# yangt1013/SPEINet

Measured on AMD Instinct MI355X. Metric: deblurred 720p frames/sec, higher is better.
Workload: dtype f16 (correlation top2)

## Files before the change

### include/speinet_hip.h

```cpp
#ifndef SPEINET_HIP_H
#define SPEINET_HIP_H

#include <stdint.h>

#ifdef __cplusplus
extern "C" {
#endif

typedef void* spei_stream_t;

#define SPEI_ACT_NONE 0
#define SPEI_ACT_RELU 1
#define SPEI_ACT_GELU 2

#define SPEI_F32 0
#define SPEI_BF16 1
#define SPEI_F16 2

#define SPEI_CONV 0
#define SPEI_CONV_TRANSPOSED 1

int spei_version(void);
const char* spei_last_error(void);
const char* spei_arch(void);
// ... 10 lines not shown
                   int W, int Cin, spei_stream_t stream);

int spei_igemm_f32(const float* a0, int lda0, int k0, const float* a1, int lda1, int k1, const float* w,
                   const float* bias, float* out, int ldo, const float* residual, int ldr,
                   const float* rowscale, int Hin, int Win, int Hout, int Wout, int N, int ksize, int stride,
                   int pad, int mode, int act, spei_stream_t stream);

int spei_igemm_f32_batched(const float* a0, int lda0, int k0, const float* a1, int lda1, int k1, const float* w,
                           const float* bias, float* out, int ldo, const float* residual, int ldr,
                           const float* rowscale, int Hin, int Win, int Hout, int Wout, int N, int ksize, int stride,
                           int pad, int mode, int act, int batch, spei_stream_t stream);

int spei_conv_slab16(int fmt, const void* a0, int lda0, int k0, const void* a1, int lda1, int k1, int a_fmt,
                     const void* wfrag_hi, const void* wfrag_lo, const float* bias, void* out, int ldo, int out_fmt,
                     const float* residual, int ldr, const float* rowscale, int Hin, int Win, int Hout, int Wout,
                     int N, int ksize, int stride, int pad, int act, int ln_input, spei_stream_t stream);

int spei_conv_slab16_batched(int fmt, const void* a0, int k0, int a_fmt, const void* wfrag, const void* wfrag_lo, const float* bias,
                             void* out, int out_fmt, const float* residual, int batch, int Hin, int Win, int Hout, int Wout, int N,
                             int ksize, int stride, int pad, int act, spei_stream_t stream);

int spei_conv32_ws16(int fmt, const void* a, int a_fmt, const void* wfrag, const float* bias, void* out, int out_fmt, int batch,
                     int H, int W, int act, spei_stream_t stream);

int spei_conv64_ws16(int fmt, const void* a, int a_fmt, const void* wfrag, const float* bias, void* out, int out_fmt, int batch,
                     int H, int W, int act, spei_stream_t stream);

int spei_mlp_fused16(int fmt, const float* x, float* out, const void* w1_frag, const float* b1, const void* w2_frag,
                     const float* b2, int64_t M, spei_stream_t stream);

int spei_convt2_slab16(int fmt, const void* a0, int lda0, int k0, int a_fmt, const void* wfrag00, const void* wfrag01,
                       const void* wfrag10, const void* wfrag11, const float* bias, void* out, int ldo, int out_fmt,
                       int Hin, int Win, int N, int act, spei_stream_t stream);

int spei_convt2_slab16x3(const float* a0, int lda0, int k0, const void* const* whi4, const void* const* wlo4, const float* bias,
                         float* out, int ldo, int Hin, int Win, int N, int act, spei_stream_t stream);

int spei_conv3x3_256_pipe16(int fmt, const float* x, const void* w_frag, const float* bias, const float* residual, float* out,
                            int batch, int H, int W, spei_stream_t stream);

int spei_conv5_out_slab16(int fmt, const void* in, int ldi, int in_fmt, const void* wfrag, const float* bias32, float* out_chw,
                          int H, int W, spei_stream_t stream);

int spei_attn_fused16(int fmt, const float* x, float* out, const void* yhat, const void* wq_frag, const float* bq,
                      const void* wkv_frag, const float* bkv, const void* wproj_frag, const float* bproj,
                      const float* relbias, int H, int W, int shift, spei_stream_t stream);
// ... 233 lines not shown
```

### speinet_amd/csrc/common.h

```cpp
#pragma once
#include <hip/hip_runtime.h>
#include <stdint.h>
#include <stdio.h>
#include "../../include/speinet_hip.h"

void spei_set_error(const char* fmt, ...);

#define SPEI_REQUIRE(cond, ...)            \
    do {                                   \
        if (!(cond)) {                     \
            spei_set_error(__VA_ARGS__);   \
            return -1;                     \
        }                                  \
    } while (0)

#define SPEI_CHECK_LAUNCH(name)                                                          \
    do {                                                                                 \
        hipError_t e__ = hipGetLastError();                                              \
        if (e__ != hipSuccess) {                                                         \
            spei_set_error("%s: launch failed: %s", name, hipGetErrorString(e__));       \
            return -2;                                                                   \
        }                                                                                \
    } while (0)

// ... 108 lines not shown
__device__ __forceinline__ typename lpv<LP>::x4 to_lp4(f32x4 v) {
    typename lpv<LP>::x4 h;
    h[0] = to_lp<LP>(v[0]); h[1] = to_lp<LP>(v[1]); h[2] = to_lp<LP>(v[2]); h[3] = to_lp<LP>(v[3]);
    return h;
}
typedef unsigned u32x4 __attribute__((ext_vector_type(4)));

template <int CTRL>
__device__ __forceinline__ float dpp_quad(float v) {
    return __int_as_float(__builtin_amdgcn_update_dpp(0, __float_as_int(v), CTRL, 0xF, 0xF, true));
}
__device__ __forceinline__ void quad_transpose4(float& a0, float& a1, float& a2, float& a3, int t) {
    const bool b0 = t & 1, b1 = t & 2;
    float s = b0 ? a0 : a1, r = dpp_quad<0xB1>(s);
    if (b0) a0 = r; else a1 = r;
    s = b0 ? a2 : a3; r = dpp_quad<0xB1>(s);
    if (b0) a2 = r; else a3 = r;
    s = b1 ? a0 : a2; r = dpp_quad<0x4E>(s);
    if (b1) a0 = r; else a2 = r;
    s = b1 ? a1 : a3; r = dpp_quad<0x4E>(s);
    if (b1) a1 = r; else a3 = r;
}

__device__ __forceinline__ float spei_gray_px(float r, float g, float b) {
    return __fmaf_rn(0.114f, b, __fmaf_rn(0.2989f, r, 0.587f * g)) / 255.0f;
}
```

### speinet_amd/csrc/conv32_ws16.hip

```cpp
#include "common.h"

namespace {

constexpr int C = 32, KS = 5, PAD = 2, NTAP = KS * KS;
constexpr int TH = 16, TW = 32;
constexpr int IH = TH + KS - 1, IW = TW + KS - 1;
constexpr int PITCH = 2 * C + 16;
constexpr int SLAB = IH * IW * PITCH;
constexpr int NTHR = 256, RT = 4;

struct WsParams {
    const void* a;
    const void* wfrag;
    const float* bias;
    void* out;
    int H, W, batch, act;
    int tiles_x, tiles_y, total;
    long long* stamps;
};

__device__ __forceinline__ void mfma_aw(f32x16& acc, const lpv<_Float16>::x8& w, const lpv<_Float16>::x8& b) {
    asm volatile("v_mfma_f32_32x32x16_f16 %0, %1, %2, %0" : "+v"(acc) : "a"(w), "v"(b));
}
__device__ __forceinline__ void mfma_aw(f32x16& acc, const lpv<__bf16>::x8& w, const lpv<__bf16>::x8& b) {
    asm volatile("v_mfma_f32_32x32x16_bf16 %0, %1, %2, %0" : "+v"(acc) : "a"(w), "v"(b));
}

template <typename TA> struct Chunk { static constexpr int CPP = sizeof(TA) == 4 ? 8 : 4; };

template <typename LP, typename TA, typename TO>
__global__ __launch_bounds__(NTHR, 1) void conv32_ws_kernel(const WsParams p) {
    typedef typename lpv<LP>::x8 lp8;
    typedef typename lpv<LP>::x4 lp4;
    constexpr int CPP = Chunk<TA>::CPP;
    constexpr int NCH = IH * IW * CPP;
    constexpr int NIT = (NCH + NTHR - 1) / NTHR;
    constexpr int NPH = sizeof(TA) == 4 ? 2 : 1;
    constexpr int NITH = (NIT + NPH - 1) / NPH;
    extern __shared__ __attribute__((aligned(16))) unsigned char smem[];

    const int tid = threadIdx.x, lane = tid & 63, wave = tid >> 6;
    const int fr = lane & 31, fk = lane >> 5;

    lp8 wreg[NTAP][2];
    {
        const LP* wp = static_cast<const LP*>(p.wfrag) + lane * 8;
#pragma unroll
        for (int t = 0; t < NTAP; ++t)
#pragma unroll
            for (int s = 0; s < 2; ++s) wreg[t][s] = *reinterpret_cast<const lp8*>(wp + (t * 2 + s) * 512);
    }
    float biasv[16];
#pragma unroll
    for (int r = 0; r < 16; ++r) biasv[r] = p.bias ? p.bias[8 * (r >> 2) + 4 * fk + (r & 3)] : 0.f;

    typedef u32x4 stage_t;
    stage_t sreg[NITH];
    const size_t map_elems = (size_t)p.H * p.W * C;
    const int per_map = p.tiles_x * p.tiles_y;

    auto tile_origin = [&](int t, int& b, int& oy0, int& ox0) {
        b = t / per_map;
        const int r = t - b * per_map;
        const int ty = r / p.tiles_x;
        oy0 = ty * TH;
        ox0 = (r - ty * p.tiles_x) * TW;
    };
    constexpr int PPI = NTHR / CPP, E = 16 / (int)sizeof(TA);
    const int p0 = tid / CPP, sub = tid - p0 * CPP;
    const int iy0 = p0 / IW, ix0 = p0 - iy0 * IW;
    const int lds0 = p0 * PITCH + sub * (sizeof(TA) == 4 ? 8 : 16);
    auto advance = [](int& iy, int& ix) {
        ix += PPI % IW;
        iy += PPI / IW;
        if (ix >= IW) { ix -= IW; ++iy; }
    };
    auto load_slab = [&](int t, int ph) {
        int b, oy0, ox0;
        tile_origin(t, b, oy0, ox0);
        const TA* base = static_cast<const TA*>(p.a) + (size_t)b * map_elems + sub * E;
// ... 11 lines not shown
    auto store_slab = [&](int t, int buf, int ph, int lo, int hi) {
        int b, oy0, ox0;
        tile_origin(t, b, oy0, ox0);
        unsigned char* sl = smem + buf * SLAB + lds0;
        int iy = iy0, ix = ix0;
#pragma unroll
        for (int it = 0; it < NIT; ++it) {
            if (it >= ph * NITH + lo && it < ph * NITH + hi && it < (ph + 1) * NITH && iy < IH) {
                const int j = it - ph * NITH;
                const bool ok = ((unsigned)(oy0 - PAD + iy) < (unsigned)p.H) & ((unsigned)(ox0 - PAD + ix) < (unsigned)p.W);
                if constexpr (sizeof(TA) == 4) {
                    const f32x4 v = __builtin_bit_cast(f32x4, sreg[j]);
                    lp4 h = to_lp4<LP>(v);
                    if (!ok) h = lp4{(LP)0.f, (LP)0.f, (LP)0.f, (LP)0.f};
                    *reinterpret_cast<lp4*>(sl + it * PPI * PITCH) = h;
                } else {
                    *reinterpret_cast<stage_t*>(sl + it * PPI * PITCH) = ok ? sreg[j] : stage_t{0u, 0u, 0u, 0u};
                }
            }
            advance(iy, ix);
        }
    };

    int t = blockIdx.x;
    if (t >= p.total) return;
#pragma unroll
    for (int ph = 0; ph < NPH; ++ph) {
        load_slab(t, ph);
        store_slab(t, 0, ph, 0, NITH);
    }
    lds_barrier();

    int boff[RT];
#pragma unroll
    for (int i = 0; i < RT; ++i) boff[i] = ((wave * RT + i) * IW + fr) * PITCH + fk * 16;

    int buf = 0;
    for (; t < p.total; t += gridDim.x, buf ^= 1) {
        const int tn = t + gridDim.x;
        const bool more = tn < p.total;
        const int tl = more ? tn : t;
        const bool st_ = t == (int)blockIdx.x + (int)gridDim.x;
        if (st_) SPEI_STAMP(p.stamps, 0);
        load_slab(tl, 0);
        if (st_) SPEI_STAMP(p.stamps, 1);
        __builtin_amdgcn_sched_barrier(0);

        const unsigned char* sl = smem + buf * SLAB;
        f32x16 acc[RT];
#pragma unroll
        for (int i = 0; i < RT; ++i)
#pragma unroll
            for (int r = 0; r < 16; ++r) acc[i][r] = biasv[r];
        lp8 bq[3][RT];
        auto step_off = [](int step) { const int tap = step >> 1; return ((tap / KS) * IW + (tap % KS)) * PITCH + (step & 1) * 32; };
#pragma unroll
        for (int d = 0; d < 2; ++d)
#pragma unroll
            for (int i = 0; i < RT; ++i) bq[d][i] = *reinterpret_cast<const lp8*>(sl + boff[i] + step_off(d));
#pragma unroll
        for (int step = 0; step < NTAP * 2; ++step) {
            const int tap = step >> 1, s2 = step & 1;
            if (step + 2 < NTAP * 2) {
#pragma unroll
                for (int i = 0; i < RT; ++i) bq[(step + 2) % 3][i] = *reinterpret_cast<const lp8*>(sl + boff[i] + step_off(step + 2));
            }
#pragma unroll
            for (int i = 0; i < RT; ++i) mfma_aw(acc[i], wreg[tap][s2], bq[step % 3][i]);
            if (NPH == 2 && step == NTAP) {
                store_slab(tl, buf ^ 1, 0, 0, NITH);
                load_slab(tl, 1);
            }
            if (NPH == 1 && step >= NTAP && ((step - NTAP) & 1) == 0 && (step - NTAP) / 2 < NITH)
                store_slab(tl, buf ^ 1, 0, (step - NTAP) / 2, (step - NTAP) / 2 + 1);
        }

        if (st_) SPEI_STAMP(p.stamps, 2);
        {
            int b, oy0, ox0;
            tile_origin(t, b, oy0, ox0);
            TO* ob = static_cast<TO*>(p.out) + (size_t)b * map_elems;
            const int ox = ox0 + fr;
#pragma unroll
            for (int i = 0; i < RT; ++i) {
                const int oy = oy0 + wave * RT + i;
                if (oy < p.H && ox < p.W) {
                    TO* o = ob + ((size_t)oy * p.W + ox) * C + 4 * fk;
#pragma unroll
                    for (int g = 0; g < 4; ++g) {
                        f32x4 v = {acc[i][4 * g], acc[i][4 * g + 1], acc[i][4 * g + 2], acc[i][4 * g + 3]};
                        if (p.act == SPEI_ACT_RELU) v = f32x4{fmaxf(v[0], 0.f), fmaxf(v[1], 0.f), fmaxf(v[2], 0.f), fmaxf(v[3], 0.f)};
                        if constexpr (sizeof(TO) == 4) *reinterpret_cast<f32x4*>(o + 8 * g) = v;
                        else *reinterpret_cast<lp4*>(o + 8 * g) = to_lp4<LP>(v);
                    }
                }
            }
        }
        if (st_) SPEI_STAMP(p.stamps, 3);
        if (NPH == 2) store_slab(tl, buf ^ 1, 1, 0, NITH);
        else store_slab(tl, buf ^ 1, 0, (NTAP + 1) / 2, NITH);
        if (st_) SPEI_STAMP(p.stamps, 4);
        lds_barrier();
        if (st_) SPEI_STAMP(p.stamps, 5);
    }
}

template <typename LP>
int launch_ws(const WsParams& p, int a16, int o16, hipStream_t st) {
    const size_t lds = 2 * (size_t)SLAB;
    const int cus = spei_num_cus();
    const dim3 grid(p.total < cus ? p.total : cus);
    if (a16 && o16) {
        ensure_dyn_lds<&conv32_ws_kernel<LP, LP, LP>>(lds);
        hipLaunchKernelGGL((conv32_ws_kernel<LP, LP, LP>), grid, dim3(NTHR), lds, st, p);
    } else if (!a16 && o16) {
        ensure_dyn_lds<&conv32_ws_kernel<LP, float, LP>>(lds);
        hipLaunchKernelGGL((conv32_ws_kernel<LP, float, LP>), grid, dim3(NTHR), lds, st, p);
    } else if (a16 && !o16) {
        ensure_dyn_lds<&conv32_ws_kernel<LP, LP, float>>(lds);
        hipLaunchKernelGGL((conv32_ws_kernel<LP, LP, float>), grid, dim3(NTHR), lds, st, p);
    } else {
        ensure_dyn_lds<&conv32_ws_kernel<LP, float, float>>(lds);
        hipLaunchKernelGGL((conv32_ws_kernel<LP, float, float>), grid, dim3(NTHR), lds, st, p);
    }
    return 0;
}

}

extern "C" int spei_conv32_ws16(int fmt, const void* a, int a_fmt, const void* wfrag, const float* bias, void* out, int out_fmt, int batch,
                                int H, int W, int act, spei_stream_t stream) {
    SPEI_REQUIRE(a && wfrag && out, "spei_conv32_ws16: null pointer");
    SPEI_REQUIRE((fmt == SPEI_BF16 || fmt == SPEI_F16) && (a_fmt == SPEI_F32 || a_fmt == fmt) && (out_fmt == SPEI_F32 || out_fmt == fmt),
                 "spei_conv32_ws16: fmt=%d a_fmt=%d out_fmt=%d", fmt, a_fmt, out_fmt);
    SPEI_REQUIRE(batch >= 1 && H > 0 && W > 0 && (int64_t)batch * cdiv(H, TH) * cdiv(W, TW) < (1ll << 30) && (int64_t)H * W < (1ll << 26),
                 "spei_conv32_ws16: batch=%d of %dx%d", batch, H, W);
    SPEI_REQUIRE(act == SPEI_ACT_NONE || act == SPEI_ACT_RELU, "spei_conv32_ws16: act=%d", act);
    SPEI_REQUIRE(((uintptr_t)a | (uintptr_t)wfrag | (uintptr_t)out) % 16 == 0 && a != out, "spei_conv32_ws16: 16-byte alignment, out must not be the input");
    WsParams p;
    p.a = a; p.wfrag = wfrag; p.bias = bias; p.out = out; p.H = H; p.W = W; p.batch = batch; p.act = act;
    p.tiles_x = cdiv(W, TW); p.tiles_y = cdiv(H, TH); p.total = batch * p.tiles_x * p.tiles_y;
    p.stamps = spei_stamp_buffer();
    hipStream_t st = (hipStream_t)stream;
    const int a16 = a_fmt != SPEI_F32, o16 = out_fmt != SPEI_F32;
    const int rc = fmt == SPEI_F16 ? launch_ws<_Float16>(p, a16, o16, st) : launch_ws<__bf16>(p, a16, o16, st);
    if (rc) return rc;
    SPEI_CHECK_LAUNCH("spei_conv32_ws16");
    return 0;
}
```

### speinet_amd/csrc/resblock.hip

```cpp
#include "common.h"

namespace {

constexpr int GATE_TR16 = 16;
constexpr int GATE_TR32 = 8;
__host__ __device__ inline int gate_tr(bool lp) { return lp ? GATE_TR16 : GATE_TR32; }
__host__ __device__ inline int gate_tc(int C) { return 256 / (C / 8); }

struct GateWs {
    float* rowpmax;
    float* rowpsum;
    float* colpmax;
    float* colpsum;
    float* tilesum;
    int ntx, nty;
};
__host__ __device__ inline GateWs carve(float* ws, int H, int W, int C, bool lp) {
    GateWs g;
    g.ntx = (W + gate_tc(C) - 1) / gate_tc(C);
    g.nty = (H + gate_tr(lp) - 1) / gate_tr(lp);
    g.rowpmax = ws;
    g.rowpsum = g.rowpmax + (size_t)g.ntx * H * C;
    g.colpmax = g.rowpsum + (size_t)g.ntx * H * C;
    g.colpsum = g.colpmax + (size_t)g.nty * W * C;
// ... 287 lines not shown
                }
            }
        }
        g2[i] = fmaf(acc, hc_bn[0], hc_bn[1]);
    }
}

template <typename T>
__global__ __launch_bounds__(256) void resblock_apply_kernel(const float* __restrict__ x, const T* __restrict__ x1,
                                                             const float* __restrict__ s, const float* __restrict__ g1,
                                                             const float* __restrict__ g2, const float* __restrict__ extra,
                                                             float* __restrict__ out, int ldo, int H, int W, int C) {
    const int cg = C / 4;
    const int64_t total = (int64_t)H * W * cg;
    {
        const size_t b = blockIdx.y;
        x += b * H * W * C; x1 += b * H * W * C; out += b * H * W * ldo;
        s += b * C; g1 += b * H * C; g2 += b * W * C;
    }
    for (int64_t i = (int64_t)blockIdx.x * 256 + threadIdx.x; i < total; i += (int64_t)gridDim.x * 256) {
        const int c = (int)(i % cg) * 4;
        const int64_t pix = i / cg;
        const int xx = (int)(pix % W), yy = (int)(pix / W);
        const float4 a = *reinterpret_cast<const float4*>(x + pix * C + c);
        const f32x4 bv = ld4<T>(x1 + pix * C + c);
        const float4 b = make_float4(bv[0], bv[1], bv[2], bv[3]);
        const float4 sv = *reinterpret_cast<const float4*>(s + c);
        const float4 u = *reinterpret_cast<const float4*>(g1 + (size_t)yy * C + c);
        const float4 v = *reinterpret_cast<const float4*>(g2 + (size_t)xx * C + c);
        float4 o;
        o.x = (b.x * sv.x + (b.x * u.x + b.x * v.x)) + a.x;
        o.y = (b.y * sv.y + (b.y * u.y + b.y * v.y)) + a.y;
        o.z = (b.z * sv.z + (b.z * u.z + b.z * v.z)) + a.z;
        o.w = (b.w * sv.w + (b.w * u.w + b.w * v.w)) + a.w;
        if (extra) {
            const float4 e = *reinterpret_cast<const float4*>(extra + pix * C + c);
            o.x += e.x; o.y += e.y; o.z += e.z; o.w += e.w;
        }
        *reinterpret_cast<float4*>(out + pix * ldo + c) = o;
    }
}

}

extern "C" int64_t spei_gate_ws_floats(int H, int W, int C) {
    if (C != 32 && C != 64 && C != 128) return 0;
    const int64_t ntx = (W + gate_tc(C) - 1) / gate_tc(C), nty = (H + GATE_TR32 - 1) / GATE_TR32;
    return 2 * ntx * H * C + 2 * nty * W * C + ntx * nty * C;
}

static int resblock_gates_run(const void* x1, int x1_fmt, int batch, int H, int W, int C, const float* se_w1, const float* se_b1,
                              const float* se_w2, const float* se_b2, const float* cw_w, const float* cw_bn,
                              const float* hc_w, const float* hc_bn, float* s, float* g1, float* g2, float* ws,
                              spei_stream_t stream) {
    SPEI_REQUIRE(batch >= 1 && batch <= 65535, "spei_resblock_gates_batched: batch=%d", batch);
    SPEI_REQUIRE(x1 && se_w1 && se_b1 && se_w2 && se_b2 && cw_w && cw_bn && hc_w && hc_bn && s && g1 && g2 && ws,
                 "spei_resblock_gates: null pointer");
    SPEI_REQUIRE(C == 32 || C == 64 || C == 128, "spei_resblock_gates: C=%d (32/64/128 built)", C);
    SPEI_REQUIRE(H > 0 && W > 0, "spei_resblock_gates: empty map");
    SPEI_REQUIRE(((uintptr_t)x1 | (uintptr_t)ws) % 16 == 0, "spei_resblock_gates: 16-byte alignment required");
    hipStream_t st = (hipStream_t)stream;
    SPEI_REQUIRE(x1_fmt == SPEI_F32 || x1_fmt == SPEI_BF16 || x1_fmt == SPEI_F16, "spei_resblock_gates: x1_fmt=%d", x1_fmt);
// ... 64 lines not shown
```

### speinet_amd/engine.py

```python
from __future__ import annotations

import contextlib
from functools import partial

import torch

from .ops import ACT_GELU, ACT_RELU, CONV_T, BMap, Ctx, FMap


def _resblocks(ctx: Ctx, f: FMap, blocks, extra=None, out=None) -> FMap:
    n = len(blocks)
    for i, pk in enumerate(blocks):
        last = i == n - 1
        f = ctx.resblock(f, pk, extra=extra if last else None, out=out if last else None)
    return f


def in_block(ctx: Ctx, frame: torch.Tensor, pk: dict) -> FMap:
    ctx = ctx.for_stage("enc")
    return _resblocks(ctx, ctx.conv5_in(frame, pk["head_w"], pk["head_b"]), pk["blocks"])


def enc_stage(ctx: Ctx, f: FMap, pk: dict, extra=None, out=None) -> FMap:
    ctx = ctx.for_stage("enc")
    n = pk["head_b"].numel()
    f = ctx.igemm(f, pk["head_w"], pk["head_b"], n, ksize=5, stride=2, act=ACT_RELU)
    return _resblocks(ctx, f, pk["blocks"], extra, out)


def enc(ctx: Ctx, frame: torch.Tensor, P: dict, extra=None, out=None) -> FMap:
    return enc_stage(ctx, enc_stage(ctx, in_block(ctx, frame, P["inBlock"]), P["encoder_first"]), P["encoder_second"], extra, out)


def enc_batched(ctx: Ctx, frames: list, P: dict):
    ctx = ctx.for_stage("enc")
    assert ctx.batched_available()
    b, (h, w) = len(frames), frames[0].shape[-2:]
    ib = P["inBlock"]
    lv1 = BMap.empty(b, h, w, ib["head_b"].numel(), frames[0].device)
    lib_in = lambda i: ctx.conv5_in(frames[i], ib["head_w"], ib["head_b"], out=lv1.map(i))
    for i in range(b):
        lib_in(i)
    for pk in ib["blocks"]:
        lv1 = ctx.resblock_batched(lv1, pk)
    levels = [lv1]
    f = lv1
    for name in ("encoder_first", "encoder_second"):
        st = P[name]
        f = ctx.igemm_batched(f, st["head_w"], st["head_b"], st["head_b"].numel(), 5, stride=2, act=ACT_RELU)
        for pk in st["blocks"]:
            f = ctx.resblock_batched(f, pk)
        levels.append(f)
    return levels


def dec_stage(ctx: Ctx, f: FMap, pk: dict) -> FMap:
    f = _resblocks(ctx, f, pk["blocks"])
    return ctx.for_stage("convt").igemm(f, pk["tail_w"], pk["tail_b"], pk["tail_b"].numel(), ksize=3, stride=2, mode=CONV_T, act=ACT_RELU)


class SwinX:

    def __init__(self, ctx: Ctx, f_mid: FMap, sw: dict):
        ctx = ctx.for_stage("swin")
        self.f_mid = f_mid
        self.x_first = ctx.igemm(f_mid, sw["conv_first_w"], sw["conv_first_b"], 256, ksize=3)
        self.xt0 = ctx.layernorm(self.x_first.t, sw["pe_g"], sw["pe_b"])
# ... 358 lines not shown
```

### speinet_amd/ops.py

```python
from __future__ import annotations

import ctypes as C
import dataclasses
from typing import Optional

import numpy as np
import torch

from . import _lib, y4m
from . import light as _light
from .pack import BF16, F16, F32, LP_DTYPE, PackedW, fmt_of

ACT_NONE, ACT_RELU, ACT_GELU = 0, 1, 2
CONV, CONV_T = 0, 1

PRECISIONS = ("f32", "bf16x3", "bf16", "f16")
CORR_PRECISIONS = ("bf16x3", "single", "top2")
_CORR_ALIASES = {"bf16": "single", "bf16r": "top2", "f16": "single"}


class FMap:
    __slots__ = ("t", "H", "W", "C", "ld", "off")

    def __init__(self, t: torch.Tensor, H: int, W: int, C_: int, off: int = 0):
# ... 34 lines not shown
        return FMap(x.permute(1, 2, 0).reshape(h * w, c).contiguous().float(), h, w, c)


class BMap:
    __slots__ = ("t", "B", "H", "W", "C")

    def __init__(self, t: torch.Tensor, B: int, H: int, W: int, C_: int):
        assert t.is_cuda and t.is_contiguous() and t.shape == (B * H * W, C_)
        self.t, self.B, self.H, self.W, self.C = t, B, H, W, C_

    @staticmethod
    def empty(B: int, H: int, W: int, C_: int, device, dtype=torch.float32) -> "BMap":
        return BMap(torch.empty(B * H * W, C_, device=device, dtype=dtype), B, H, W, C_)

    @property
    def fmt(self) -> int:
        return fmt_of(self.t.dtype)

    def map(self, b: int) -> FMap:
        n = self.H * self.W
        return FMap(self.t[b * n:(b + 1) * n], self.H, self.W, self.C)


def _vp(p) -> C.c_void_p:
    return C.c_void_p(p)


class _timed:
    def __init__(self, ctx: "Ctx", name: str):
        self.on = ctx.profile is not None and name in ctx.profile
        self.ctx, self.name = ctx, name

    def __enter__(self):
        if self.on:
            self.s = torch.cuda.Event(enable_timing=True)
            self.e = torch.cuda.Event(enable_timing=True)
            self.s.record(torch.cuda.current_stream(self.ctx.device))
        return self

    def __exit__(self, *a):
        if self.on:
            self.e.record(torch.cuda.current_stream(self.ctx.device))
            self.ctx.profile[self.name].append((self.s, self.e))
        return False


def _tensor_bytes(x) -> int:
    t = x.t if hasattr(x, "t") else x
    return t.numel() * t.element_size() if torch.is_tensor(t) else 0


def _conv_sub(method: str, a, k, out):
    if method == "conv5_in":
        return "level1", 2.0 * 25 * 3 * 32 * a[0].shape[-2] * a[0].shape[-1], _tensor_bytes(a[0]) + _tensor_bytes(out)
    if method == "conv5_out":
        return "level1", 2.0 * 25 * 32 * 3 * a[0].H * a[0].W, _tensor_bytes(a[0]) + 12 * a[0].H * a[0].W
    src, n = a[0], a[3]
    ks = a[4] if len(a) > 4 else k.get("ksize", 1)
    if n == 32 and src.C == 32 and ks == 5 and k.get("stride", a[5] if len(a) > 5 else 1) == 1:
        maps = getattr(src, "B", 1)
        return "level1", 2.0 * 25 * 32 * 32 * maps * src.H * src.W, _tensor_bytes(src) + _tensor_bytes(out)
    return "rest", 0.0, 0


def _family(name: str):
    def deco(fn):
        def wrapper(self, *a, **k):
            pr = self.profile
            if pr is None or "families" not in pr:
                return fn(self, *a, **k)
            st = torch.cuda.current_stream(self.device)
            s_, e_ = torch.cuda.Event(enable_timing=True), torch.cuda.Event(enable_timing=True)
            s_.record(st)
            out = fn(self, *a, **k)
            e_.record(st)
            pr["families"].setdefault(name, []).append((s_, e_))
            if name == "conv":
                sub, fl, by = _conv_sub(fn.__name__, a, k, out)
                rec = pr.setdefault("conv_sub", {}).setdefault(sub, {"events": [], "flops": 0.0, "bytes": 0})
# ... 304 lines not shown

@dataclasses.dataclass(frozen=True, slots=True, eq=False)
class Ctx:
    ACT_NONE, ACT_RELU, ACT_GELU = ACT_NONE, ACT_RELU, ACT_GELU
    CONV, CONV_T = CONV, CONV_T
    SPLIT_STAGES = ("glue", "dec2")

    precision: str = "f32"
    corr_precision: str = "bf16x3"
    device: Optional[torch.device] = None
    bf16_storage: bool = True
    x1_bf16: bool = True
    fuse_mlp: bool = True
    fuse_attn: bool = True
    commute_upconv: bool = True
    commute_any: bool = False
    corr_bf16: bool = True
    corr_diag: bool = True
    split_decode: bool = True
    batch_enc: bool = True
    attn_win4: bool = True
    conv32_ws: bool = True
    conv64_ws: Optional[bool] = None
    conv3_pipe: bool = True
    stage: Optional[dict] = None
    profile: Optional[dict] = None
    capture: Optional[dict] = None

    def __post_init__(self):
        put = object.__setattr__
        if self.precision not in PRECISIONS:
            raise ValueError(f"unknown precision {self.precision!r}")
        put(self, "corr_precision", _CORR_ALIASES.get(self.corr_precision, self.corr_precision))
        if self.corr_precision not in CORR_PRECISIONS:
            raise ValueError(f"unknown correlation precision {self.corr_precision!r}")
        cur = torch.cuda.current_device() if torch.cuda.is_available() else 0
        device = torch.device("cuda", cur) if self.device is None else torch.device(self.device)
        if device.type != "cuda":
            raise RuntimeError("speinet_amd runs on MI355X only (HIP kernels); there is no CPU path")
        put(self, "device", torch.device("cuda", cur) if device.index is None else device)
        for k in _BOOL_KNOBS:
            if type(getattr(self, k)) is not bool:
                put(self, k, bool(getattr(self, k)))
        if self.conv64_ws is not None:
            put(self, "conv64_ws", bool(self.conv64_ws))
        put(self, "stage", dict(self.stage) if self.stage else {})
# ... 196 lines not shown
            w = PackedW(w.reshape(1, *w.shape), x.device)
        n = w.shape[1]
        if out is None:
            out = torch.empty(m, n, device=x.device, dtype=out_dtype)
        self.igemm(FMap(x, m, 1, k), w, b, n, act=act, ln_input=ln_input,
                   residual=FMap(residual, m, 1, n) if residual is not None else None, out=FMap(out, m, 1, n))
        return out

    @_family("streaming")
    def resblock_gates(self, x1: FMap, pk: dict):
        dev = x1.t.device
        lib = _lib.lib()
        tp = self._tp
        assert x1.off == 0 and x1.ld == x1.C
        s = torch.empty(x1.C, device=dev)
        g1 = torch.empty(x1.H, x1.C, device=dev)
        g2 = torch.empty(x1.W, x1.C, device=dev)
        ws = torch.empty(lib.spei_gate_ws_floats(x1.H, x1.W, x1.C), device=dev)
        _lib.check(lib.spei_resblock_gates(self._fp(x1), x1.fmt, x1.H, x1.W, x1.C, tp(pk["se_w1"]), tp(pk["se_b1"]), tp(pk["se_w2"]),
                                           tp(pk["se_b2"]), tp(pk["cw_w"]), tp(pk["cw_bn"]), tp(pk["hc_w"]), tp(pk["hc_bn"]),
                                           tp(s), tp(g1), tp(g2), tp(ws), self._stream()), "spei_resblock_gates")
        return s, g1, g2

    def resblock(self, x: FMap, pk: dict, extra: Optional[FMap] = None, out: Optional[FMap] = None) -> FMap:
        idt = self.inter_dtype()
        c = x.C
        assert x.off == 0 and x.ld == c
        t = self.igemm(x, pk["w1"], pk["b1"], c, ksize=5, act=ACT_RELU, out_dtype=idt)
        x1 = self.igemm(t, pk["w2"], pk["b2"], c, ksize=5, out_dtype=idt if self.x1_bf16 else torch.float32)
        s, g1, g2 = self.resblock_gates(x1, pk)
        if out is None:
            out = FMap.empty(x.H, x.W, c, x.t.device)
        if extra is not None:
            assert extra.off == 0 and extra.ld == c
        self._apply(x, x1, s, g1, g2, extra, out, c)
        return out

    @_family("streaming")
    def _apply(self, x, x1, s, g1, g2, extra, out, c):
        _lib.check(_lib.lib().spei_resblock_apply(self._fp(x), self._fp(x1), x1.fmt, self._tp(s), self._tp(g1), self._tp(g2),
                                                  self._fp(extra), self._fp(out), out.ld, x.H, x.W, c, self._stream()),
                   "spei_resblock_apply")

    def batched_available(self) -> bool:
        return self.batched_kernels() and self.x1_bf16 and self.bf16_storage and self.batch_enc

    def conv32_ws_available(self) -> bool:
        return self.lp16 and self.conv32_ws

    def conv64_ws_available(self) -> bool:
        return self.lp16 and (self.conv32_ws if self.conv64_ws is None else self.conv64_ws)

    def batched_kernels(self) -> bool:
        return self.lp16

    @_family("conv")
    def igemm_batched(self, a: BMap, w, bias: torch.Tensor, N: int, ksize: int, stride: int = 1, act: int = ACT_NONE,
                      out_dtype=torch.float32, residual: Optional[BMap] = None, out: Optional[BMap] = None) -> BMap:
        assert self.batched_kernels() and not torch.is_tensor(w) and w.fhi is not None
        pad = ksize // 2
        ho, wo = (a.H + 2 * pad - ksize) // stride + 1, (a.W + 2 * pad - ksize) // stride + 1
        assert tuple(w.shape) == (ksize * ksize, N, a.C) and a.t.dtype in (torch.float32, LP_DTYPE[self.fmt])
        if out is None:
            out = BMap.empty(a.B, ho, wo, N, a.t.device, out_dtype)
        assert (out.B, out.H, out.W, out.C) == (a.B, ho, wo, N) and out.t.data_ptr() != a.t.data_ptr()
        if residual is not None:
            assert (residual.B, residual.H, residual.W, residual.C) == (a.B, ho, wo, N) and residual.t.dtype == torch.float32
            assert residual.t.data_ptr() != a.t.data_ptr()
        tp = self._tp
        if self._persistent_conv(a, w, bias, N, ksize, stride, act, residual, out, a.B):
            return out
        _lib.check(_lib.lib().spei_conv_slab16_batched(self.fmt, tp(a.t), a.C, a.fmt, tp(w.frag(self.fmt)), _vp(0), tp(bias), tp(out.t), out.fmt,
                                                       tp(residual.t) if residual is not None else _vp(0), a.B, a.H, a.W, ho, wo, N, ksize,
                                                       stride, pad, act, self._stream()),
                   "spei_conv_slab16_batched")
        return out

    def resblock_batched(self, x: BMap, pk: dict) -> BMap:
        idt = self.inter_dtype()
        c, dev = x.C, x.t.device
        lib = _lib.lib()
        tp = self._tp
        t = self.igemm_batched(x, pk["w1"], pk["b1"], c, 5, act=ACT_RELU, out_dtype=idt)
        x1 = self.igemm_batched(t, pk["w2"], pk["b2"], c, 5, out_dtype=idt)
        del t
        return self._gates_apply_batched(x, x1, pk)

    @_family("streaming")
    def _gates_apply_batched(self, x: BMap, x1: BMap, pk: dict) -> BMap:
        c, dev = x.C, x.t.device
        lib = _lib.lib()
        tp = self._tp
        s = torch.empty(x.B, c, device=dev)
        g1 = torch.empty(x.B, x.H, c, device=dev)
        g2 = torch.empty(x.B, x.W, c, device=dev)
        ws = torch.empty(x.B * lib.spei_gate_ws_floats(x.H, x.W, c), device=dev)
        _lib.check(lib.spei_resblock_gates_batched(tp(x1.t), x1.fmt, x.B, x.H, x.W, c, tp(pk["se_w1"]), tp(pk["se_b1"]), tp(pk["se_w2"]),
                                                   tp(pk["se_b2"]), tp(pk["cw_w"]), tp(pk["cw_bn"]), tp(pk["hc_w"]), tp(pk["hc_bn"]),
                                                   tp(s), tp(g1), tp(g2), tp(ws), self._stream()), "spei_resblock_gates_batched")
        out = BMap.empty(x.B, x.H, x.W, c, dev)
        _lib.check(lib.spei_resblock_apply_batched(tp(x.t), tp(x1.t), x1.fmt, tp(s), tp(g1), tp(g2), tp(out.t), x.B, x.H, x.W, c,
                                                   self._stream()), "spei_resblock_apply_batched")
        return out

    def ln_fused_available(self) -> bool:
        return self.precision != "f32"

    def attn_fused_available(self) -> bool:
        return self.lp16 and self.fuse_attn and self.bf16_storage

    def mlp_fused_available(self) -> bool:
        return self.lp16 and self.fuse_mlp

    def swin_multi_available(self) -> bool:
        return self.attn_fused_available() and self.attn_win4 and self.mlp_fused_available() and self.batched_kernels()

    @_family("swin")
    def attn_fused(self, x: torch.Tensor, yhat: torch.Tensor, bk: dict, H: int, W: int, shift: int, out: torch.Tensor) -> torch.Tensor:
        assert x.shape[0] % (H * W) == 0 and x.shape[1] == 256 and x.dtype == torch.float32 and out.shape == x.shape and out.dtype == torch.float32
        f = self.fmt
        assert yhat.shape == x.shape and yhat.dtype == LP_DTYPE[f]
        tp = self._tp
# ... 136 lines not shown
```

Baseline: 41.27.

## Fuse resblock gated-apply into next block's first conv32 weight-stationary kernel

Defers the resblock gate-apply (x + x1*(s+g1+g2)) so that the next resblock's first 5x5 conv computes it on the fly while staging its input slab. The gated sum is written to LDS as the conv input and also stored to global as the new residual x. The staging goes through a register ring, and gate vectors are double-buffered in LDS. This removes one full-resolution streaming kernel and its read-then-reread of x per resblock. In exchange the conv loader reads more bytes per pixel (fp32 x plus x1 and the gate rows), register pressure rises, and the gated sum is recomputed on halo pixels.

Measured after the change: 41.63, median of 6. No clear change (+0.9%).

```diff
diff --git a/include/speinet_hip.h b/include/speinet_hip.h
--- a/include/speinet_hip.h
+++ b/include/speinet_hip.h
@@ -56,6 +56,9 @@
 
 int spei_conv32_ws16(int fmt, const void* a, int a_fmt, const void* wfrag, const float* bias, void* out, int out_fmt, int batch,
                      int H, int W, int act, spei_stream_t stream);
+
+int spei_conv32_ws16_gated(int fmt, const float* x, const void* x1, const float* s, const float* g1, const float* g2, const void* wfrag,
+                           const float* bias, float* xo, void* t, int batch, int H, int W, int act, spei_stream_t stream);
 
 int spei_conv64_ws16(int fmt, const void* a, int a_fmt, const void* wfrag, const float* bias, void* out, int out_fmt, int batch,
                      int H, int W, int act, spei_stream_t stream);
diff --git a/speinet_amd/csrc/common.h b/speinet_amd/csrc/common.h
--- a/speinet_amd/csrc/common.h
+++ b/speinet_amd/csrc/common.h
@@ -154,6 +154,17 @@
     if (b1) a1 = r; else a3 = r;
 }
 
+__device__ __forceinline__ f32x4 spei_gated_sum4(f32x4 x, f32x4 x1, f32x4 s, f32x4 g1, f32x4 g2) {
+#pragma clang fp contract(off)
+    f32x4 o;
+#pragma unroll
+    for (int e = 0; e < 4; ++e) {
+        const float p2 = x1[e] * g2[e];
+        o[e] = __builtin_fmaf(x1[e], s[e], __builtin_fmaf(x1[e], g1[e], p2)) + x[e];
+    }
+    return o;
+}
+
 __device__ __forceinline__ float spei_gray_px(float r, float g, float b) {
     return __fmaf_rn(0.114f, b, __fmaf_rn(0.2989f, r, 0.587f * g)) / 255.0f;
 }
diff --git a/speinet_amd/csrc/conv32_ws16.hip b/speinet_amd/csrc/conv32_ws16.hip
--- a/speinet_amd/csrc/conv32_ws16.hip
+++ b/speinet_amd/csrc/conv32_ws16.hip
@@ -8,6 +8,9 @@
 constexpr int PITCH = 2 * C + 16;
 constexpr int SLAB = IH * IW * PITCH;
 constexpr int NTHR = 256, RT = 4;
+constexpr int G2_OFF = IH * C * 4, GS_OFF = G2_OFF + IW * C * 4, GATE = GS_OFF + C * 4;
+constexpr int NGC = GATE / 16;
+constexpr int BIAS_OFF = 2 * SLAB + 2 * GATE;
 
 struct WsParams {
     const void* a;
@@ -17,7 +20,14 @@
     int H, W, batch, act;
     int tiles_x, tiles_y, total;
     long long* stamps;
+    const void* x1;
+    const float* s;
+    const float* g1;
+    const float* g2;
+    float* xo;
 };
+
+typedef unsigned u32x2 __attribute__((ext_vector_type(2)));
 
 __device__ __forceinline__ void mfma_aw(f32x16& acc, const lpv<_Float16>::x8& w, const lpv<_Float16>::x8& b) {
     asm volatile("v_mfma_f32_32x32x16_f16 %0, %1, %2, %0" : "+v"(acc) : "a"(w), "v"(b));
@@ -28,8 +38,9 @@
 
 template <typename TA> struct Chunk { static constexpr int CPP = sizeof(TA) == 4 ? 8 : 4; };
 
-template <typename LP, typename TA, typename TO>
+template <typename LP, typename TA, typename TO, bool GATED = false>
 __global__ __launch_bounds__(NTHR, 1) void conv32_ws_kernel(const WsParams p) {
+    static_assert(!GATED || sizeof(TA) == 4, "gated input: x is fp32");
     typedef typename lpv<LP>::x8 lp8;
     typedef typename lpv<LP>::x4 lp4;
     constexpr int CPP = Chunk<TA>::CPP;
@@ -37,6 +48,7 @@
     constexpr int NIT = (NCH + NTHR - 1) / NTHR;
     constexpr int NPH = sizeof(TA) == 4 ? 2 : 1;
     constexpr int NITH = (NIT + NPH - 1) / NPH;
+    constexpr int RING = 8;
     extern __shared__ __attribute__((aligned(16))) unsigned char smem[];
 
     const int tid = threadIdx.x, lane = tid & 63, wave = tid >> 6;
@@ -53,9 +65,17 @@
     float biasv[16];
 #pragma unroll
     for (int r = 0; r < 16; ++r) biasv[r] = p.bias ? p.bias[8 * (r >> 2) + 4 * fk + (r & 3)] : 0.f;
+    if constexpr (GATED) {
+#pragma unroll
+        for (int g = 0; g < 4; ++g)
+            if (fr == 0 && wave == 0)
+                *reinterpret_cast<f32x4*>(smem + BIAS_OFF + (8 * g + 4 * fk) * 4) = f32x4{biasv[4 * g], biasv[4 * g + 1], biasv[4 * g + 2], biasv[4 * g + 3]};
+    }
 
     typedef u32x4 stage_t;
-    stage_t sreg[NITH];
+    stage_t sreg[GATED ? RING : NITH];
+    u32x2 s1reg[GATED ? RING : 1];
+    stage_t greg[2];
     const size_t map_elems = (size_t)p.H * p.W * C;
     const int per_map = p.tiles_x * p.tiles_y;
 
@@ -113,12 +133,80 @@
         }
     };
 
+    int p0t = p0;
+    auto load_chunk = [&](int t, int it, int slot) {
+        int b, oy0, ox0;
+        tile_origin(t, b, oy0, ox0);
+        const int pix = p0t + it * PPI, iy = min(pix / IW, IH - 1), ix = pix - (pix / IW) * IW;
+        const int gy = min(max(oy0 - PAD + iy, 0), p.H - 1), gx = min(max(ox0 - PAD + ix, 0), p.W - 1);
+        const size_t off = (size_t)b * map_elems + sub * E + (gy * p.W + gx) * C;
+        sreg[slot] = *reinterpret_cast<const stage_t*>(static_cast<const float*>(p.a) + off);
+        s1reg[slot] = *reinterpret_cast<const u32x2*>(static_cast<const LP*>(p.x1) + off);
+    };
+    auto store_chunk = [&](int t, int buf, int it, int slot, bool wr) {
+        int b, oy0, ox0;
+        tile_origin(t, b, oy0, ox0);
+        const int pix = p0t + it * PPI, iy = pix / IW, ix = pix - iy * IW;
+        if (iy < IH) {
+            const unsigned char* gt = smem + 2 * SLAB + buf * GATE + sub * 16;
+            const bool ok = ((unsigned)(oy0 - PAD + iy) < (unsigned)p.H) & ((unsigned)(ox0 - PAD + ix) < (unsigned)p.W);
+            const lp4 h1 = __builtin_bit_cast(lp4, s1reg[slot]);
+            const f32x4 b1 = {(float)h1[0], (float)h1[1], (float)h1[2], (float)h1[3]};
+            const f32x4 v = spei_gated_sum4(__builtin_bit_cast(f32x4, sreg[slot]), b1, *reinterpret_cast<const f32x4*>(gt + GS_OFF),
+                                            *reinterpret_cast<const f32x4*>(gt + iy * (C * 4)), *reinterpret_cast<const f32x4*>(gt + G2_OFF + ix * (C * 4)));
+            lp4 h = to_lp4<LP>(v);
+            if (!ok) h = lp4{(LP)0.f, (LP)0.f, (LP)0.f, (LP)0.f};
+            *reinterpret_cast<lp4*>(smem + buf * SLAB + lds0 + it * PPI * PITCH) = h;
+            if (ok && wr && (unsigned)(iy - PAD) < (unsigned)TH && (unsigned)(ix - PAD) < (unsigned)TW)
+                *reinterpret_cast<f32x4*>(p.xo + (size_t)b * map_elems + sub * E + ((oy0 - PAD + iy) * p.W + (ox0 - PAD + ix)) * C) = v;
+        }
+    };
+    auto load_gates = [&](int t, int k0, int k1) {
+        int b, oy0, ox0;
+        tile_origin(t, b, oy0, ox0);
+#pragma unroll
+        for (int k = k0; k < k1; ++k) {
+            const int c = min(tid + k * NTHR, NGC - 1);
+            const bool r1 = c < G2_OFF / 16, r2 = c < GS_OFF / 16;
+            const int l = r1 ? oy0 - PAD + (c >> 3) : ox0 - PAD + ((c - G2_OFF / 16) >> 3);
+            const int line = r2 ? min(max(l, 0), (r1 ? p.H : p.W) - 1) : 0;
+            const float* base = r1 ? p.g1 + (size_t)b * p.H * C : r2 ? p.g2 + (size_t)b * p.W * C : p.s + (size_t)b * C;
+            const float* src = base + line * C + (c & 7) * 4;
+            greg[k] = *reinterpret_cast<const stage_t*>(src);
+        }
+    };
+    auto store_gates = [&](int buf, int k0, int k1) {
+#pragma unroll
+        for (int k = k0; k < k1; ++k)
+            if (tid + k * NTHR < NGC) *reinterpret_cast<stage_t*>(smem + 2 * SLAB + buf * GATE + (tid + k * NTHR) * 16) = greg[k];
+    };
+
     int t = blockIdx.x;
     if (t >= p.total) return;
-#pragma unroll
-    for (int ph = 0; ph < NPH; ++ph) {
-        load_slab(t, ph);
-        store_slab(t, 0, ph, 0, NITH);
+    if constexpr (GATED) {
+        load_gates(t, 0, 2);
+        store_gates(0, 0, 2);
+        lds_barrier();
+#pragma unroll
+        for (int r = 0; r < NIT; r += RING) {
+#pragma unroll
+            for (int j = 0; j < RING; ++j)
+                if (r + j < NIT) load_chunk(t, r + j, j);
+#pragma unroll
+            for (int j = 0; j < RING; ++j)
+                if (r + j < NIT) store_chunk(t, 0, r + j, j, true);
+        }
+        const int tn = t + (int)gridDim.x < p.total ? t + (int)gridDim.x : t;
+        load_gates(tn, 0, 2);
+        store_gates(1, 0, 2);
+#pragma unroll
+        for (int j = 0; j < RING; ++j) load_chunk(tn, j, j);
+    } else {
+#pragma unroll
+        for (int ph = 0; ph < NPH; ++ph) {
+            load_slab(t, ph);
+            store_slab(t, 0, ph, 0, NITH);
+        }
     }
     lds_barrier();
 
@@ -132,8 +220,14 @@
         const bool more = tn < p.total;
         const int tl = more ? tn : t;
         const bool st_ = t == (int)blockIdx.x + (int)gridDim.x;
+        const int tl2 = t + 2 * (int)gridDim.x < p.total ? t + 2 * (int)gridDim.x : t;
         if (st_) SPEI_STAMP(p.stamps, 0);
-        load_slab(tl, 0);
+        if constexpr (GATED) {
+            asm volatile("" : "+v"(p0t));
+            load_gates(tl2, 0, 1);
+        } else {
+            load_slab(tl, 0);
+        }
         if (st_) SPEI_STAMP(p.stamps, 1);
         __builtin_amdgcn_sched_barrier(0);
 
@@ -142,15 +236,17 @@
 #pragma unroll
         for (int i = 0; i < RT; ++i)
 #pragma unroll
-            for (int r = 0; r < 16; ++r) acc[i][r] = biasv[r];
+            for (int r = 0; r < 16; ++r) {
+                if constexpr (GATED) acc[i][r] = reinterpret_cast<const float*>(smem + BIAS_OFF)[8 * (r >> 2) + 4 * fk + (r & 3)];
+                else acc[i][r] = biasv[r];
+            }
         lp8 bq[3][RT];
         auto step_off = [](int step) { const int tap = step >> 1; return ((tap / KS) * IW + (tap % KS)) * PITCH + (step & 1) * 32; };
 #pragma unroll
         for (int d = 0; d < 2; ++d)
 #pragma unroll
             for (int i = 0; i < RT; ++i) bq[d][i] = *reinterpret_cast<const lp8*>(sl + boff[i] + step_off(d));
-#pragma unroll
-        for (int step = 0; step < NTAP * 2; ++step) {
+        auto mfma_step = [&](int step) __attribute__((always_inline)) {
             const int tap = step >> 1, s2 = step & 1;
             if (step + 2 < NTAP * 2) {
 #pragma unroll
@@ -158,12 +254,25 @@
             }
 #pragma unroll
             for (int i = 0; i < RT; ++i) mfma_aw(acc[i], wreg[tap][s2], bq[step % 3][i]);
-            if (NPH == 2 && step == NTAP) {
+        };
+#pragma unroll
+        for (int step = 0; step < NTAP * 2; ++step) {
+            mfma_step(step);
+            if (!GATED && NPH == 2 && step == NTAP) {
                 store_slab(tl, buf ^ 1, 0, 0, NITH);
                 load_slab(tl, 1);
             }
             if (NPH == 1 && step >= NTAP && ((step - NTAP) & 1) == 0 && (step - NTAP) / 2 < NITH)
                 store_slab(tl, buf ^ 1, 0, (step - NTAP) / 2, (step - NTAP) / 2 + 1);
+            if constexpr (GATED) {
+                if ((step & 1) && step / 2 < NIT) {
+                    const int e = step / 2;
+                    store_chunk(tl, buf ^ 1, e, e % RING, more);
+                    load_chunk(e + RING < NIT ? tl : tl2, e + RING < NIT ? e + RING : e % RING, e % RING);
+                }
+                if (step == 16) { store_gates(buf, 0, 1); load_gates(tl2, 1, 2); }
+                if (step == 32) store_gates(buf, 1, 2);
+            }
         }
 
         if (st_) SPEI_STAMP(p.stamps, 2);
@@ -188,8 +297,8 @@
             }
         }
         if (st_) SPEI_STAMP(p.stamps, 3);
-        if (NPH == 2) store_slab(tl, buf ^ 1, 1, 0, NITH);
-        else store_slab(tl, buf ^ 1, 0, (NTAP + 1) / 2, NITH);
+        if (!GATED && NPH == 2) store_slab(tl, buf ^ 1, 1, 0, NITH);
+        else if (!GATED) store_slab(tl, buf ^ 1, 0, (NTAP + 1) / 2, NITH);
         if (st_) SPEI_STAMP(p.stamps, 4);
         lds_barrier();
         if (st_) SPEI_STAMP(p.stamps, 5);
@@ -217,6 +326,14 @@
     return 0;
 }
 
+template <typename LP>
+void launch_ws_gated(const WsParams& p, hipStream_t st) {
+    const size_t lds = BIAS_OFF + C * sizeof(float);
+    const int cus = spei_num_cus();
+    ensure_dyn_lds<&conv32_ws_kernel<LP, float, LP, true>>(lds);
+    hipLaunchKernelGGL((conv32_ws_kernel<LP, float, LP, true>), dim3(p.total < cus ? p.total : cus), dim3(NTHR), lds, st, p);
+}
+
 }
 
 extern "C" int spei_conv32_ws16(int fmt, const void* a, int a_fmt, const void* wfrag, const float* bias, void* out, int out_fmt, int batch,
@@ -232,6 +349,7 @@
     p.a = a; p.wfrag = wfrag; p.bias = bias; p.out = out; p.H = H; p.W = W; p.batch = batch; p.act = act;
     p.tiles_x = cdiv(W, TW); p.tiles_y = cdiv(H, TH); p.total = batch * p.tiles_x * p.tiles_y;
     p.stamps = spei_stamp_buffer();
+    p.x1 = nullptr; p.s = p.g1 = p.g2 = nullptr; p.xo = nullptr;
     hipStream_t st = (hipStream_t)stream;
     const int a16 = a_fmt != SPEI_F32, o16 = out_fmt != SPEI_F32;
     const int rc = fmt == SPEI_F16 ? launch_ws<_Float16>(p, a16, o16, st) : launch_ws<__bf16>(p, a16, o16, st);
@@ -239,3 +357,25 @@
     SPEI_CHECK_LAUNCH("spei_conv32_ws16");
     return 0;
 }
+
+extern "C" int spei_conv32_ws16_gated(int fmt, const float* x, const void* x1, const float* s, const float* g1, const float* g2, const void* wfrag,
+                                      const float* bias, float* xo, void* t, int batch, int H, int W, int act, spei_stream_t stream) {
+    SPEI_REQUIRE(x && x1 && s && g1 && g2 && wfrag && xo && t, "spei_conv32_ws16_gated: null pointer");
+    SPEI_REQUIRE(fmt == SPEI_BF16 || fmt == SPEI_F16, "spei_conv32_ws16_gated: fmt=%d", fmt);
+    SPEI_REQUIRE(batch >= 1 && H > 0 && W > 0 && (int64_t)batch * cdiv(H, TH) * cdiv(W, TW) < (1ll << 30) && (int64_t)H * W < (1ll << 26),
+                 "spei_conv32_ws16_gated: batch=%d of %dx%d", batch, H, W);
+    SPEI_REQUIRE(act == SPEI_ACT_NONE || act == SPEI_ACT_RELU, "spei_conv32_ws16_gated: act=%d", act);
+    SPEI_REQUIRE(((uintptr_t)x | (uintptr_t)x1 | (uintptr_t)s | (uintptr_t)g1 | (uintptr_t)g2 | (uintptr_t)wfrag | (uintptr_t)xo | (uintptr_t)t) % 16 == 0,
+                 "spei_conv32_ws16_gated: 16-byte alignment");
+    SPEI_REQUIRE((const void*)xo != (const void*)x && (const void*)xo != x1 && (const void*)xo != t && (const void*)t != (const void*)x && t != x1,
+                 "spei_conv32_ws16_gated: xo and t must not be an input or each other (halo pixels re-read x and x1)");
+    WsParams p;
+    p.a = x; p.wfrag = wfrag; p.bias = bias; p.out = t; p.H = H; p.W = W; p.batch = batch; p.act = act;
+    p.tiles_x = cdiv(W, TW); p.tiles_y = cdiv(H, TH); p.total = batch * p.tiles_x * p.tiles_y;
+    p.stamps = spei_stamp_buffer();
+    p.x1 = x1; p.s = s; p.g1 = g1; p.g2 = g2; p.xo = xo;
+    if (fmt == SPEI_F16) launch_ws_gated<_Float16>(p, (hipStream_t)stream);
+    else launch_ws_gated<__bf16>(p, (hipStream_t)stream);
+    SPEI_CHECK_LAUNCH("spei_conv32_ws16_gated");
+    return 0;
+}
diff --git a/speinet_amd/csrc/resblock.hip b/speinet_amd/csrc/resblock.hip
--- a/speinet_amd/csrc/resblock.hip
+++ b/speinet_amd/csrc/resblock.hip
@@ -333,22 +333,14 @@
         const int c = (int)(i % cg) * 4;
         const int64_t pix = i / cg;
         const int xx = (int)(pix % W), yy = (int)(pix / W);
-        const float4 a = *reinterpret_cast<const float4*>(x + pix * C + c);
-        const f32x4 bv = ld4<T>(x1 + pix * C + c);
-        const float4 b = make_float4(bv[0], bv[1], bv[2], bv[3]);
-        const float4 sv = *reinterpret_cast<const float4*>(s + c);
-        const float4 u = *reinterpret_cast<const float4*>(g1 + (size_t)yy * C + c);
-        const float4 v = *reinterpret_cast<const float4*>(g2 + (size_t)xx * C + c);
-        float4 o;
-        o.x = (b.x * sv.x + (b.x * u.x + b.x * v.x)) + a.x;
-        o.y = (b.y * sv.y + (b.y * u.y + b.y * v.y)) + a.y;
-        o.z = (b.z * sv.z + (b.z * u.z + b.z * v.z)) + a.z;
-        o.w = (b.w * sv.w + (b.w * u.w + b.w * v.w)) + a.w;
-        if (extra) {
-            const float4 e = *reinterpret_cast<const float4*>(extra + pix * C + c);
-            o.x += e.x; o.y += e.y; o.z += e.z; o.w += e.w;
-        }
-        *reinterpret_cast<float4*>(out + pix * ldo + c) = o;
+        const f32x4 a = *reinterpret_cast<const f32x4*>(x + pix * C + c);
+        const f32x4 b = ld4<T>(x1 + pix * C + c);
+        const f32x4 sv = *reinterpret_cast<const f32x4*>(s + c);
+        const f32x4 u = *reinterpret_cast<const f32x4*>(g1 + (size_t)yy * C + c);
+        const f32x4 v = *reinterpret_cast<const f32x4*>(g2 + (size_t)xx * C + c);
+        f32x4 o = spei_gated_sum4(a, b, sv, u, v);
+        if (extra) o += *reinterpret_cast<const f32x4*>(extra + pix * C + c);
+        *reinterpret_cast<f32x4*>(out + pix * ldo + c) = o;
     }
 }
 
diff --git a/speinet_amd/engine.py b/speinet_amd/engine.py
--- a/speinet_amd/engine.py
+++ b/speinet_amd/engine.py
@@ -12,7 +12,7 @@
     n = len(blocks)
     for i, pk in enumerate(blocks):
         last = i == n - 1
-        f = ctx.resblock(f, pk, extra=extra if last else None, out=out if last else None)
+        f = ctx.resblock(f, pk, extra=extra if last else None, out=out if last else None, nxt=None if last else blocks[i + 1])
     return f
 
 
@@ -41,8 +41,8 @@
     lib_in = lambda i: ctx.conv5_in(frames[i], ib["head_w"], ib["head_b"], out=lv1.map(i))
     for i in range(b):
         lib_in(i)
-    for pk in ib["blocks"]:
-        lv1 = ctx.resblock_batched(lv1, pk)
+    for i, pk in enumerate(ib["blocks"]):
+        lv1 = ctx.resblock_batched(lv1, pk, nxt=ib["blocks"][i + 1] if i + 1 < len(ib["blocks"]) else None)
     levels = [lv1]
     f = lv1
     for name in ("encoder_first", "encoder_second"):
diff --git a/speinet_amd/ops.py b/speinet_amd/ops.py
--- a/speinet_amd/ops.py
+++ b/speinet_amd/ops.py
@@ -80,6 +80,13 @@
         return FMap(self.t[b * n:(b + 1) * n], self.H, self.W, self.C)
 
 
+class GatedSum:
+    __slots__ = ("x", "x1", "s", "g1", "g2")
+
+    def __init__(self, x, x1, s: torch.Tensor, g1: torch.Tensor, g2: torch.Tensor):
+        self.x, self.x1, self.s, self.g1, self.g2 = x, x1, s, g1, g2
+
+
 def _vp(p) -> C.c_void_p:
     return C.c_void_p(p)
 
@@ -113,6 +120,10 @@
         return "level1", 2.0 * 25 * 3 * 32 * a[0].shape[-2] * a[0].shape[-1], _tensor_bytes(a[0]) + _tensor_bytes(out)
     if method == "conv5_out":
         return "level1", 2.0 * 25 * 32 * 3 * a[0].H * a[0].W, _tensor_bytes(a[0]) + 12 * a[0].H * a[0].W
+    if method == "_conv1_gated":
+        g = a[0]
+        return ("level1", 2.0 * 25 * 32 * 32 * getattr(g.x, "B", 1) * g.x.H * g.x.W,
+                _tensor_bytes(g.x) + _tensor_bytes(g.x1) + sum(_tensor_bytes(o) for o in out))
     src, n = a[0], a[3]
     ks = a[4] if len(a) > 4 else k.get("ksize", 1)
     if n == 32 and src.C == 32 and ks == 5 and k.get("stride", a[5] if len(a) > 5 else 1) == 1:
@@ -463,6 +474,7 @@
     attn_win4: bool = True
     conv32_ws: bool = True
     conv64_ws: Optional[bool] = None
+    defer_apply: bool = True
     conv3_pipe: bool = True
     stage: Optional[dict] = None
     profile: Optional[dict] = None
@@ -705,13 +717,19 @@
                                            tp(s), tp(g1), tp(g2), tp(ws), self._stream()), "spei_resblock_gates")
         return s, g1, g2
 
-    def resblock(self, x: FMap, pk: dict, extra: Optional[FMap] = None, out: Optional[FMap] = None) -> FMap:
+    def resblock(self, x, pk: dict, extra: Optional[FMap] = None, out: Optional[FMap] = None, nxt: Optional[dict] = None):
         idt = self.inter_dtype()
-        c = x.C
-        assert x.off == 0 and x.ld == c
-        t = self.igemm(x, pk["w1"], pk["b1"], c, ksize=5, act=ACT_RELU, out_dtype=idt)
+        if isinstance(x, GatedSum):
+            x, t = self._conv1_gated(x, pk)
+            c = x.C
+        else:
+            c = x.C
+            assert x.off == 0 and x.ld == c
+            t = self.igemm(x, pk["w1"], pk["b1"], c, ksize=5, act=ACT_RELU, out_dtype=idt)
         x1 = self.igemm(t, pk["w2"], pk["b2"], c, ksize=5, out_dtype=idt if self.x1_bf16 else torch.float32)
         s, g1, g2 = self.resblock_gates(x1, pk)
+        if nxt is not None and extra is None and out is None and self.defer_ok(x, nxt):
+            return GatedSum(x, x1, s, g1, g2)
         if out is None:
             out = FMap.empty(x.H, x.W, c, x.t.device)
         if extra is not None:
@@ -730,6 +748,29 @@
 
     def conv32_ws_available(self) -> bool:
         return self.lp16 and self.conv32_ws
+
+    def defer_ok(self, x, nxt: dict) -> bool:
+        w = nxt["w1"]
+        return (self.defer_apply and self.conv32_ws_available() and self.x1_bf16 and self.bf16_storage and x.C == 32
+                and x.t.dtype == torch.float32 and (getattr(x, "ld", 32), getattr(x, "off", 0)) == (32, 0)
+                and not torch.is_tensor(w) and w.fhi is not None and tuple(w.shape) == (25, 32, 32))
+
+    @_family("conv")
+    def _conv1_gated(self, g: GatedSum, pk: dict):
+        x, x1 = g.x, g.x1
+        dev, idt = x.t.device, self.inter_dtype()
+        if isinstance(x, BMap):
+            batch, ptr = x.B, lambda m: self._tp(m.t)
+            xo, t = BMap.empty(x.B, x.H, x.W, 32, dev), BMap.empty(x.B, x.H, x.W, 32, dev, idt)
+        else:
+            batch, ptr = 1, self._fp
+            xo, t = FMap.empty(x.H, x.W, 32, dev), FMap.empty(x.H, x.W, 32, dev, idt)
+        assert x.C == 32 and x1.fmt == self.fmt and idt == LP_DTYPE[self.fmt]
+        tp = self._tp
+        _lib.check(_lib.lib().spei_conv32_ws16_gated(self.fmt, ptr(x), ptr(x1), tp(g.s), tp(g.g1), tp(g.g2), tp(pk["w1"].frag(self.fmt)),
+                                                     tp(pk["b1"]), ptr(xo), ptr(t), batch, x.H, x.W, ACT_RELU, self._stream()),
+                   "spei_conv32_ws16_gated")
+        return xo, t
 
     def conv64_ws_available(self) -> bool:
         return self.lp16 and (self.conv32_ws if self.conv64_ws is None else self.conv64_ws)
@@ -759,18 +800,20 @@
                    "spei_conv_slab16_batched")
         return out
 
-    def resblock_batched(self, x: BMap, pk: dict) -> BMap:
+    def resblock_batched(self, x, pk: dict, nxt: Optional[dict] = None):
         idt = self.inter_dtype()
-        c, dev = x.C, x.t.device
-        lib = _lib.lib()
-        tp = self._tp
-        t = self.igemm_batched(x, pk["w1"], pk["b1"], c, 5, act=ACT_RELU, out_dtype=idt)
+        if isinstance(x, GatedSum):
+            x, t = self._conv1_gated(x, pk)
+            c = x.C
+        else:
+            c = x.C
+            t = self.igemm_batched(x, pk["w1"], pk["b1"], c, 5, act=ACT_RELU, out_dtype=idt)
         x1 = self.igemm_batched(t, pk["w2"], pk["b2"], c, 5, out_dtype=idt)
         del t
-        return self._gates_apply_batched(x, x1, pk)
+        return self._gates_apply_batched(x, x1, pk, nxt is not None and self.defer_ok(x, nxt))
 
     @_family("streaming")
-    def _gates_apply_batched(self, x: BMap, x1: BMap, pk: dict) -> BMap:
+    def _gates_apply_batched(self, x: BMap, x1: BMap, pk: dict, defer: bool = False):
         c, dev = x.C, x.t.device
         lib = _lib.lib()
         tp = self._tp
@@ -781,6 +824,8 @@
         _lib.check(lib.spei_resblock_gates_batched(tp(x1.t), x1.fmt, x.B, x.H, x.W, c, tp(pk["se_w1"]), tp(pk["se_b1"]), tp(pk["se_w2"]),
                                                    tp(pk["se_b2"]), tp(pk["cw_w"]), tp(pk["cw_bn"]), tp(pk["hc_w"]), tp(pk["hc_bn"]),
                                                    tp(s), tp(g1), tp(g2), tp(ws), self._stream()), "spei_resblock_gates_batched")
+        if defer:
+            return GatedSum(x, x1, s, g1, g2)
         out = BMap.empty(x.B, x.H, x.W, c, dev)
         _lib.check(lib.spei_resblock_apply_batched(tp(x.t), tp(x1.t), x1.fmt, tp(s), tp(g1), tp(g2), tp(out.t), x.B, x.H, x.W, c,
                                                    self._stream()), "spei_resblock_apply_batched")
```
